# batd-htplus/intool-rag

Hardware: AMD Instinct MI355X
Metric: queries/sec, exact top-10 inner-product search, 1M x 1024-d fp32 index (higher is better)
Workload: dtype bf16 x bf16 -> f32 filter scan, f64 re-score of the f32 rows; 1 GPU; configs[1]: 1M x 1024-d synthetic unit vectors, brute-force inner-product top-10; rows=1000000, dim=1024, k=10, queries_per_pass=64, exchange=none, steps_in_flight=4, world=1, backend=none, allgather_payload_bytes_per_rank=0

## Files before the change

### intool-rag_amd/csrc/dense_plan.h

```cpp
#pragma once
#include <algorithm>
#include <cmath>
#include <cstddef>
#include <cstdint>

#include "../../include/hiprag.h"

namespace hiprag {

constexpr int kPassQ = 64;
constexpr int kMaxQ = 1024;
constexpr int kMaxKFast = 128;
constexpr int kClasses = 64;
constexpr int kNoFilterGroups = 1024;

constexpr int kStageHalf = 896;
constexpr int kThetaBack = 8;
constexpr int kCandBytes = 16;

constexpr int kWideBlocks = 8;
constexpr int kWideQTiles = 8;
constexpr int kWideKP = 4;
constexpr int kWideBufFrags = (kWideBlocks + kWideQTiles) * kWideKP * 64;
constexpr size_t kWideLds = (size_t)2 * kWideBufFrags * 16;
constexpr int kWideMinCus = 32;
constexpr int kWideMinQ = 256;

constexpr int kPipeSpareCus = 48;
constexpr int kPipeSpareCusWide = 32;

constexpr double kLaunchPasses = 4.0;
constexpr double kLaunchRefBytes = 4.096e9;
constexpr int kMinLaunchPasses = 4;

enum ScanMode : int {
    kScanQ64 = 2,
    kScanBf16 = 3,
};

using ScanShape = hipidx_scan_shape_t;

struct ScanPlan {
    bool run = false;
    bool wide = false;
    int waves = 8;
    int ring = 16;
    bool multi_pass = false;
    bool filter = false;
    int ncls = 1;
    size_t lds_bytes = 0;
    bool qtile_image = false;
};

inline int64_t ceil_div(int64_t a, int64_t b) { return (a + b - 1) / b; }

inline bool filter_on(const ScanShape& s) { return 2 * s.nblocks > kNoFilterGroups; }
inline bool uses_qtile_images(const ScanShape& s) { return s.mode == kScanBf16; }

inline int scan_waves(const ScanShape& s, int cus)
{
    return (s.mode == kScanBf16 && s.P % 32 == 0 && s.nblocks < (int64_t)cus * 8 * 9) ? 4 : 8;
}

inline bool wide_launch_on(const ScanShape& s, int nq, int cus)
{
    if (s.mode != kScanBf16 || s.wide_env == 0 || !filter_on(s) || cus < kWideMinCus) return false;
    if (s.wide_env == 1) return nq > kPassQ;
    return nq >= kWideMinQ && ceil_div(s.nblocks, kWideBlocks) >= cus;
}

inline int64_t stream_bytes_per_pass(const ScanShape& s) { return s.nblocks * s.P * (s.mode == kScanBf16 ? 512 : 1024); }
inline int64_t bytes_per_pass(const ScanShape& s, int metric, bool wide = false)
{
    return (stream_bytes_per_pass(s) + (metric == HIPRAG_METRIC_L2 ? s.nblocks * 32 * 4 : 0)) / (wide ? 4 : 1);
}

inline int launch_queries(const ScanShape& s)
{
    if (s.launch_env > 0) return std::max(kPassQ, std::min(kMaxQ, s.launch_env / kPassQ * kPassQ));
    ScanShape t = s;
    t.nblocks = std::max<int64_t>(s.nblocks, 1);
    const int np = (int)std::lround(kLaunchPasses * kLaunchRefBytes / (double)stream_bytes_per_pass(t));
    return std::max(kMinLaunchPasses, std::min(kMaxQ / kPassQ, np)) * kPassQ;
}

inline int pipe_spare_cus(const ScanShape& s, int launch_q)
{
    const int g48 = std::max(1, s.n_cu - kPipeSpareCus), g32 = std::max(1, s.n_cu - kPipeSpareCusWide);
    if (!wide_launch_on(s, launch_q, g48) || !wide_launch_on(s, launch_q, g32)) return kPipeSpareCus;
    const int64_t nrt = ceil_div(s.nblocks, kWideBlocks);
    return ceil_div(nrt, g32) < ceil_div(nrt, g48) ? kPipeSpareCusWide : kPipeSpareCus;
}

inline ScanPlan plan_scan(const ScanShape& s, int nq, int k, int cus)
{
    ScanPlan p;
    p.filter = filter_on(s);
    p.run = s.nblocks > 0 && k <= kMaxKFast;
    if (!p.run) return p;
    p.wide = wide_launch_on(s, nq, cus);
    p.waves = p.wide ? 8 : scan_waves(s, cus);
    p.multi_pass = nq > kPassQ;
    p.ring = p.wide ? 0 : (s.mode == kScanQ64 || (s.P / 2) % 16 == 0) ? 16 : 8;
    const int64_t bpw = ceil_div(s.nblocks, (int64_t)cus * p.waves);
    p.ncls = (int)std::max<int64_t>(1, std::min<int64_t>(kClasses, ceil_div(s.nblocks, bpw)));
    p.lds_bytes = p.wide ? kWideLds : (size_t)s.P * 1024 + (size_t)2 * kStageHalf * kCandBytes + 64 + (size_t)kThetaBack * 64 * 4;
    p.qtile_image = uses_qtile_images(s) && p.multi_pass;
    return p;
}

}
```

### intool-rag_amd/csrc/scan_wide.h

```cpp
#pragma once

constexpr int kWideQ = kWideQTiles * 32;
constexpr unsigned long long kWideWaitTicks = 20000ull;

constexpr int kWideBatch = 16;
constexpr int kWidePhaseT = kClasses / kWideBatch + 1;
constexpr int kWidePhaseA = kWidePhaseT + 1;

struct WidePend {
    float f[4][2], s[4][2];
    u32 mn;
    int64_t rt;
    int unit;
    int phase;
};
struct WideFlight {
    u32 ld[kWideBatch];
    u32 tc;
    u32 pos0, pos1;
};

__device__ __forceinline__ u32 wide_theta_fresh(const ScanArgs& a, int unit, int lane, bool live)
{
    u32 m = 0;
    if (live) {
        u32* s = a.slots + (size_t)unit * kClasses * 64 + lane;
        u32 mn = 0xFFFFFFFFu;
#pragma unroll 16
        for (int c = 0; c < kClasses; ++c) mn = min(mn, load_memside_u32(s + c * 64));
        if (mn != 0) atomicMax(a.thetac + unit * 64 + lane, mn);
        m = mn;
    }
    return m;
}

__device__ __forceinline__ void wide_test(const ScanArgs& a, const WidePend& P, int bh, int lane, u32 m, bool (&p0)[4], bool (&p1)[4])
{
    const int b = lane & 31;
    const u32 th0 = (u32)__shfl((int)m, b), th1 = (u32)__shfl((int)m, 32 + b);
    const int q0 = P.unit * 64 + b, q1 = q0 + 32;
    const int64_t blk0 = P.rt * kWideBlocks + 4 * bh;
#pragma unroll
    for (int i = 0; i < 4; ++i) {
        const bool there = blk0 + i < a.nblocks;
        p0[i] = there && q0 < a.nq && ord32(P.f[i][0]) >= th0;
        p1[i] = there && q1 < a.nq && ord32(P.f[i][1]) >= th1;
    }
}

__device__ __forceinline__ void wide_issue(const ScanArgs& a, const WidePend& P, WideFlight& X, int bh, int lane)
{
    const bool live = P.unit * 64 + lane < a.nq;
#pragma unroll
    for (int i = 0; i < kWideBatch; ++i) X.ld[i] = 0xFFFFFFFFu;
    X.tc = X.pos0 = X.pos1 = 0;
    if (P.phase < kWidePhaseT) {
        if (live) {
            const u32* sl = a.slots + ((size_t)P.unit * kClasses + (size_t)(P.phase - 1) * kWideBatch) * 64 + lane;
#pragma unroll
            for (int i = 0; i < kWideBatch; ++i) X.ld[i] = load_agent_u32(sl + i * 64);
        }
    }
    if (P.phase == kWidePhaseT) {
        if (live) X.tc = __hip_atomic_fetch_max(a.thetac + P.unit * 64 + lane, P.mn, __ATOMIC_RELAXED, __HIP_MEMORY_SCOPE_AGENT);
    }
    if (P.phase == kWidePhaseA) {
        bool p0[4], p1[4];
        wide_test(a, P, bh, lane, P.mn, p0, p1);
        const u32 n0 = (u32)p0[0] + (u32)p0[1] + (u32)p0[2] + (u32)p0[3], n1 = (u32)p1[0] + (u32)p1[1] + (u32)p1[2] + (u32)p1[3];
        const int q0 = P.unit * 64 + (lane & 31);
        if (n0) X.pos0 = atomicAdd(a.count + q0, n0);
        if (n1) X.pos1 = atomicAdd(a.count + q0 + 32, n1);
    }
}

__device__ __forceinline__ void wide_land(const ScanArgs& a, WidePend& P, const WideFlight& X, int bh, int lane)
{
#pragma unroll
    for (int i = 0; i < kWideBatch; ++i) P.mn = min(P.mn, X.ld[i]);
    if (P.phase == kWidePhaseT) {
        const bool live = P.unit * 64 + lane < a.nq;
        u32 m = live ? max(P.mn, X.tc) : 0u;
        if (__ballot(live && m == 0)) {
            const unsigned long long t0 = wall_clock64();
            for (int it = 0;; ++it) {
                if (live && m == 0) m = load_memside_u32(a.thetac + P.unit * 64 + lane);
                if (it && __ballot(live && m == 0)) m = max(m, wide_theta_fresh(a, P.unit, lane, live && m == 0));
                if (!__ballot(live && m == 0)) break;
                if (wall_clock64() - t0 > kWideWaitTicks) break;
                __builtin_amdgcn_s_sleep(127);
            }
        }
        P.mn = m;
    }
    if (P.phase == kWidePhaseA) {
        bool p0[4], p1[4];
        wide_test(a, P, bh, lane, P.mn, p0, p1);
        const int h = lane >> 5;
        const u32 q0 = (u32)(P.unit * 64 + (lane & 31)), q1 = q0 + 32;
        const int64_t blk0 = P.rt * kWideBlocks + 4 * bh;
        u32 pos0 = X.pos0, pos1 = X.pos1;
#pragma unroll
        for (int i = 0; i < 4; ++i) {
            const u32 gid = (u32)(2 * (blk0 + i) + h);
            if (p0[i]) {
                if (pos0 < (u32)kCandCap) a.list[(size_t)q0 * kCandCap + pos0] = Cand{pack_key(P.f[i][0], gid), P.s[i][0], q0};
                ++pos0;
            }
            if (p1[i]) {
                if (pos1 < (u32)kCandCap) a.list[(size_t)q1 * kCandCap + pos1] = Cand{pack_key(P.f[i][1], gid), P.s[i][1], q1};
                ++pos1;
            }
        }
    }
    P.phase = P.phase == kWidePhaseA ? 0 : P.phase + 1;
}

__device__ __forceinline__ void wide_drain(const ScanArgs& a, WidePend& P, int bh, int lane)
{
    while (P.phase) {
        WideFlight X;
        wide_issue(a, P, X, bh, lane);
        wide_land(a, P, X, bh, lane);
    }
}

template <int METRIC>
__device__ __forceinline__ void wide_park(const ScanArgs& a, const f32x16 (&acc)[4][2], WidePend& P, int64_t rt, int unit, int bh, int lane)
{
    const int h = lane >> 5;
    const int64_t blk0 = rt * kWideBlocks + 4 * bh;
    if (blk0 >= a.nblocks) return;
    float pm0 = -INFINITY, pm1 = -INFINITY;
#pragma unroll
    for (int i = 0; i < 4; ++i) {
        const int64_t blk = blk0 + i;
        P.f[i][0] = P.f[i][1] = P.s[i][0] = P.s[i][1] = -FLT_MAX;
        if (blk < a.nblocks) {
            f32x4 nrm[4];
            if (METRIC == HIPRAG_METRIC_L2) {
#pragma unroll
                for (int g = 0; g < 4; ++g) nrm[g] = *reinterpret_cast<const f32x4*>(a.norms + blk * kRowsPerBlock + 8 * g + 4 * h);
            }
            P.f[i][0] = block_lane_top2<METRIC>(acc[i][0], nrm, blk, h, a, P.s[i][0]);
            P.f[i][1] = block_lane_top2<METRIC>(acc[i][1], nrm, blk, h, a, P.s[i][1]);
            pm0 = fmaxf(pm0, P.f[i][0]);
            pm1 = fmaxf(pm1, P.f[i][1]);
        }
    }
    {
        const float x0 = fmaxf(pm0, __shfl_xor(pm0, 32)), x1 = fmaxf(pm1, __shfl_xor(pm1, 32));
        const float v = lane < 32 ? x0 : x1;
        const int cls = (int)((2 * rt + bh) & (kClasses - 1));
        if (unit * 64 + lane < a.nq) atomicMax(a.slots + ((size_t)unit * kClasses + cls) * 64 + lane, ord32(v));
    }
    P.mn = 0xFFFFFFFFu;
    P.rt = rt;
    P.unit = unit;
    P.phase = 1;
}

template <int METRIC>
__global__ __launch_bounds__(512) void scan_wide_kernel(ScanArgs a)
{
    extern __shared__ float4 qs[];
    const int tid = threadIdx.x, lane = tid & 63;
    const int wave = __builtin_amdgcn_readfirstlane(tid >> 6);
    __builtin_amdgcn_s_setprio(3);
    const int64_t gw = (int64_t)blockIdx.x * 8 + wave;
    if (a.stamps && lane == 0) a.stamps[2 * gw] = wall_clock64();
    if (a.gate && tid == 0) {
        const unsigned long long was = __hip_atomic_fetch_add(a.started, 1ull, __ATOMIC_RELAXED, __HIP_MEMORY_SCOPE_AGENT);
        if (was + 1 == a.target) __hip_atomic_fetch_max(a.gate, a.seq, __ATOMIC_RELAXED, __HIP_MEMORY_SCOPE_AGENT);
    }
    const int P2 = a.P / 2;
    const int KS = P2 / kWideKP;
    const int nunits = (a.nq + 63) / 64;
    const int ncol = (a.nq + kWideQ - 1) / kWideQ;
    const int64_t nrt = (a.nblocks + kWideBlocks - 1) / kWideBlocks;
    const int bh = wave & 1, qp = wave >> 1;
    const bf16x8* xh = reinterpret_cast<const bf16x8*>(a.xh);
    const bf16x8* qimg = reinterpret_cast<const bf16x8*>(a.qtile);
    bf16x8* lds = reinterpret_cast<bf16x8*>(qs);

    auto stage = [&](int64_t rt, int col, int ks, int buf) {
        bf16x8* dst = lds + buf * kWideBufFrags;
#pragma unroll
        for (int i = 0; i < 8; ++i) {
            const int c = wave + 8 * i;
            const int pc = ks * kWideKP + (c & 3);
            if (i < 4) {
                const int64_t blk = min(rt * kWideBlocks + (c >> 2), a.nblocks - 1);
                __builtin_amdgcn_global_load_lds((const void*)(xh + ((size_t)blk * P2 + pc) * 64 + lane), (scan_lds_ptr_t)(dst + c * 64), 16, 0, 0);
            } else {
                const int qt = col * kWideQTiles + ((c - 32) >> 2);
                if ((qt >> 1) < nunits)
                    __builtin_amdgcn_global_load_lds((const void*)(qimg + ((size_t)qt * P2 + pc) * 64 + lane), (scan_lds_ptr_t)(dst + c * 64), 16, 0, 0);
            }
        }
    };

    f32x16 acc[4][2];
    WidePend P;
    P.phase = 0;
    int64_t rt = blockIdx.x;
    int col = 0, ks = 0, buf = 0;
    bool have = rt < nrt;
    if (have) stage(rt, 0, 0, 0);
    while (have) {
        int64_t nr = rt;
        int nc = col, nk = ks + 1;
        if (nk == KS) {
            nk = 0;
            if (++nc == ncol) { nc = 0; nr += gridDim.x; }
        }
        const bool more = nr < nrt;
        asm volatile("s_waitcnt vmcnt(0)" ::: "memory");
        __syncthreads();
        int lane_e = lane;
        asm volatile("" : "+v"(lane_e));
        const bool pend = P.phase != 0;
        WideFlight X;
        if (pend) wide_issue(a, P, X, bh, lane_e);
        if (more) stage(nr, nc, nk, buf ^ 1);
        const int unit = col * (kWideQTiles / 2) + qp;
        if (unit < nunits) {
            if (ks == 0) {
#pragma unroll
                for (int i = 0; i < 4; ++i)
#pragma unroll
                    for (int e = 0; e < 16; ++e) { acc[i][0][e] = 0.f; acc[i][1][e] = 0.f; }
            }
            const bf16x8* A = lds + buf * kWideBufFrags + (4 * bh) * kWideKP * 64 + lane;
            const bf16x8* B = lds + buf * kWideBufFrags + (kWideBlocks + 2 * qp) * kWideKP * 64 + lane;
#pragma unroll
            for (int pc = 0; pc < kWideKP; ++pc) {
                bf16x8 av[4], bv[2];
#pragma unroll
                for (int i = 0; i < 4; ++i) av[i] = A[(i * kWideKP + pc) * 64];
#pragma unroll
                for (int j = 0; j < 2; ++j) bv[j] = B[(j * kWideKP + pc) * 64];
#pragma unroll
                for (int i = 0; i < 4; ++i) {
                    acc[i][0] = __builtin_amdgcn_mfma_f32_32x32x16_bf16(av[i], bv[0], acc[i][0], 0, 0, 0);
                    acc[i][1] = __builtin_amdgcn_mfma_f32_32x32x16_bf16(av[i], bv[1], acc[i][1], 0, 0, 0);
                }
            }
        }
        __builtin_amdgcn_sched_barrier(0);
        if (pend) wide_land(a, P, X, bh, lane_e);
        if (unit < nunits && ks == KS - 1) {
            wide_drain(a, P, bh, lane_e);
            wide_park<METRIC>(a, acc, P, rt, unit, bh, lane_e);
        }
        rt = nr; col = nc; ks = nk; have = more; buf ^= 1;
    }
    asm volatile("s_waitcnt vmcnt(0)" ::: "memory");
    wide_drain(a, P, bh, lane);
    if (a.stamps && lane == 0) a.stamps[2 * gw + 1] = wall_clock64();
}
```

Measured before the change: 391,900 queries/s.

## Replace wide-scan double buffer with deep separate row and query LDS rings

The wide scan kernel moves from a two-buffer LDS scheme with a full vmcnt(0) wait each step to separate multi-slot rings for index rows (5 slots) and query tiles (3 slots), with the k-piece per step halved. Loads are kept several steps ahead with partial vmcnt waits, LDS reads are hand-scheduled with inline ds_read and lgkmcnt waits interleaved with MFMAs, and the threshold and count atomics are issued as inline asm with counted waits, running only every other k-step. The goal is to hide global-memory latency and overlap the bookkeeping atomics with compute. In exchange the vmcnt accounting becomes fragile and depends on exact instruction counts, and theta refreshes arrive later, which can weaken filtering.

```diff
diff --git a/intool-rag_amd/csrc/dense_plan.h b/intool-rag_amd/csrc/dense_plan.h
--- a/intool-rag_amd/csrc/dense_plan.h
+++ b/intool-rag_amd/csrc/dense_plan.h
@@ -20,9 +20,13 @@
 
 constexpr int kWideBlocks = 8;
 constexpr int kWideQTiles = 8;
-constexpr int kWideKP = 4;
-constexpr int kWideBufFrags = (kWideBlocks + kWideQTiles) * kWideKP * 64;
-constexpr size_t kWideLds = (size_t)2 * kWideBufFrags * 16;
+constexpr int kWideKP = 2;
+constexpr int kWideBufFrags = kWideBlocks * kWideKP * 64;
+static_assert(kWideBlocks == kWideQTiles, "one slot size serves both rings");
+constexpr int kWideRowRing = 5;
+constexpr int kWideQRing = 3;
+constexpr size_t kWideLds = (size_t)(kWideRowRing + kWideQRing) * kWideBufFrags * 16;
+static_assert(kWideLds == 131072, "eight 16 KiB slots, one LDS object");
 constexpr int kWideMinCus = 32;
 constexpr int kWideMinQ = 256;
 
diff --git a/intool-rag_amd/csrc/scan_wide.h b/intool-rag_amd/csrc/scan_wide.h
--- a/intool-rag_amd/csrc/scan_wide.h
+++ b/intool-rag_amd/csrc/scan_wide.h
@@ -6,6 +6,18 @@
 constexpr int kWideBatch = 16;
 constexpr int kWidePhaseT = kClasses / kWideBatch + 1;
 constexpr int kWidePhaseA = kWidePhaseT + 1;
+constexpr int kWidePhaseEvery = 2;
+
+#define WIDE_DSR(dst, addr, off) asm volatile("ds_read_b128 %0, %1 offset:%2" : "=v"(dst) : "v"(addr), "n"(off) : "memory")
+#define WIDE_LGKM1(n, x) asm volatile("s_waitcnt lgkmcnt(%[c])" : "+v"(x) : [c] "n"(n) : "memory")
+#define WIDE_LGKM3(n, x, y, z) asm volatile("s_waitcnt lgkmcnt(%[c])" : "+v"(x), "+v"(y), "+v"(z) : [c] "n"(n) : "memory")
+
+#define WIDE_BAR()                                \
+    do {                                          \
+        __builtin_amdgcn_sched_barrier(0);        \
+        __builtin_amdgcn_s_barrier();             \
+        __builtin_amdgcn_sched_barrier(0);        \
+    } while (0)
 
 struct WidePend {
     float f[4][2], s[4][2];
@@ -20,6 +32,25 @@
     u32 pos0, pos1;
 };
 
+template <int I>
+__device__ __forceinline__ void wide_slot_loads(WideFlight& X, const u32* sl)
+{
+    asm volatile("global_load_dword %0, %1, off offset:%2 sc1" : "=v"(X.ld[I]) : "v"(sl), "n"(I * 256) : "memory");
+    if constexpr (I + 1 < kWideBatch) wide_slot_loads<I + 1>(X, sl);
+}
+__device__ __forceinline__ void wide_fetch_max(u32& out, u32* p, u32 v)
+{
+    asm volatile("global_atomic_umax %0, %1, %2, off sc0" : "=v"(out) : "v"(p), "v"(v) : "memory");
+}
+__device__ __forceinline__ void wide_fetch_add(u32& out, u32* p, u32 v)
+{
+    asm volatile("global_atomic_add %0, %1, %2, off sc0" : "=v"(out) : "v"(p), "v"(v) : "memory");
+}
+#define WIDE_WAIT1(younger, a) asm volatile("s_waitcnt vmcnt(%[n])" : "+v"(a) : [n] "n"(younger) : "memory")
+#define WIDE_WAIT2(younger, a, b) asm volatile("s_waitcnt vmcnt(%[n])" : "+v"(a), "+v"(b) : [n] "n"(younger) : "memory")
+#define WIDE_WAIT8(younger, r, o) \
+    asm volatile("s_waitcnt vmcnt(%[n])" : "+v"(r[o]), "+v"(r[o + 1]), "+v"(r[o + 2]), "+v"(r[o + 3]), "+v"(r[o + 4]), "+v"(r[o + 5]), "+v"(r[o + 6]), "+v"(r[o + 7]) : [n] "n"(younger) : "memory")
+
 __device__ __forceinline__ u32 wide_theta_fresh(const ScanArgs& a, int unit, int lane, bool live)
 {
     u32 m = 0;
@@ -51,35 +82,39 @@
 __device__ __forceinline__ void wide_issue(const ScanArgs& a, const WidePend& P, WideFlight& X, int bh, int lane)
 {
     const bool live = P.unit * 64 + lane < a.nq;
-#pragma unroll
-    for (int i = 0; i < kWideBatch; ++i) X.ld[i] = 0xFFFFFFFFu;
-    X.tc = X.pos0 = X.pos1 = 0;
+    const int ql = P.unit * 64 + (live ? lane : 0);
     if (P.phase < kWidePhaseT) {
-        if (live) {
-            const u32* sl = a.slots + ((size_t)P.unit * kClasses + (size_t)(P.phase - 1) * kWideBatch) * 64 + lane;
-#pragma unroll
-            for (int i = 0; i < kWideBatch; ++i) X.ld[i] = load_agent_u32(sl + i * 64);
-        }
+        wide_slot_loads<0>(X, a.slots + ((size_t)P.unit * kClasses + (size_t)(P.phase - 1) * kWideBatch) * 64 + (ql & 63));
     }
     if (P.phase == kWidePhaseT) {
-        if (live) X.tc = __hip_atomic_fetch_max(a.thetac + P.unit * 64 + lane, P.mn, __ATOMIC_RELAXED, __HIP_MEMORY_SCOPE_AGENT);
+        wide_fetch_max(X.tc, a.thetac + ql, live ? P.mn : 0u);
     }
     if (P.phase == kWidePhaseA) {
         bool p0[4], p1[4];
         wide_test(a, P, bh, lane, P.mn, p0, p1);
         const u32 n0 = (u32)p0[0] + (u32)p0[1] + (u32)p0[2] + (u32)p0[3], n1 = (u32)p1[0] + (u32)p1[1] + (u32)p1[2] + (u32)p1[3];
         const int q0 = P.unit * 64 + (lane & 31);
-        if (n0) X.pos0 = atomicAdd(a.count + q0, n0);
-        if (n1) X.pos1 = atomicAdd(a.count + q0 + 32, n1);
-    }
-}
-
-__device__ __forceinline__ void wide_land(const ScanArgs& a, WidePend& P, const WideFlight& X, int bh, int lane)
-{
-#pragma unroll
-    for (int i = 0; i < kWideBatch; ++i) P.mn = min(P.mn, X.ld[i]);
+        X.pos0 = X.pos1 = 0;
+        if (n0) wide_fetch_add(X.pos0, a.count + q0, n0);
+        if (n1) wide_fetch_add(X.pos1, a.count + q0 + 32, n1);
+    }
+}
+
+template <bool DRAIN>
+__device__ __forceinline__ void wide_land(const ScanArgs& a, WidePend& P, WideFlight& X, int bh, int lane)
+{
+    constexpr int YOUNGER = DRAIN ? 0 : 4;
+    const bool live = P.unit * 64 + lane < a.nq;
+    if (P.phase < kWidePhaseT) {
+        WIDE_WAIT8(YOUNGER, X.ld, 0);
+        WIDE_WAIT8(YOUNGER, X.ld, 8);
+        if (live) {
+#pragma unroll
+            for (int i = 0; i < kWideBatch; ++i) P.mn = min(P.mn, X.ld[i]);
+        }
+    }
     if (P.phase == kWidePhaseT) {
-        const bool live = P.unit * 64 + lane < a.nq;
+        WIDE_WAIT1(YOUNGER, X.tc);
         u32 m = live ? max(P.mn, X.tc) : 0u;
         if (__ballot(live && m == 0)) {
             const unsigned long long t0 = wall_clock64();
@@ -94,6 +129,7 @@
         P.mn = m;
     }
     if (P.phase == kWidePhaseA) {
+        WIDE_WAIT2(YOUNGER, X.pos0, X.pos1);
         bool p0[4], p1[4];
         wide_test(a, P, bh, lane, P.mn, p0, p1);
         const int h = lane >> 5;
@@ -121,7 +157,7 @@
     while (P.phase) {
         WideFlight X;
         wide_issue(a, P, X, bh, lane);
-        wide_land(a, P, X, bh, lane);
+        wide_land<true>(a, P, X, bh, lane);
     }
 }
 
@@ -183,77 +219,106 @@
     const bf16x8* qimg = reinterpret_cast<const bf16x8*>(a.qtile);
     bf16x8* lds = reinterpret_cast<bf16x8*>(qs);
 
-    auto stage = [&](int64_t rt, int col, int ks, int buf) {
-        bf16x8* dst = lds + buf * kWideBufFrags;
-#pragma unroll
-        for (int i = 0; i < 8; ++i) {
-            const int c = wave + 8 * i;
-            const int pc = ks * kWideKP + (c & 3);
-            if (i < 4) {
-                const int64_t blk = min(rt * kWideBlocks + (c >> 2), a.nblocks - 1);
-                __builtin_amdgcn_global_load_lds((const void*)(xh + ((size_t)blk * P2 + pc) * 64 + lane), (scan_lds_ptr_t)(dst + c * 64), 16, 0, 0);
-            } else {
-                const int qt = col * kWideQTiles + ((c - 32) >> 2);
-                if ((qt >> 1) < nunits)
-                    __builtin_amdgcn_global_load_lds((const void*)(qimg + ((size_t)qt * P2 + pc) * 64 + lane), (scan_lds_ptr_t)(dst + c * 64), 16, 0, 0);
-            }
-        }
+    auto advance = [&](int64_t& rt, int& col, int& ks) -> bool {
+        if (++ks < KS) return false;
+        ks = 0;
+        if (++col == ncol) { col = 0; rt += gridDim.x; }
+        return true;
+    };
+    struct Stream { const bf16x8* p; u32 d; };
+    auto row_stream = [&](int64_t rt) {
+        const int64_t b0 = min(rt * kWideBlocks + (wave >> 1), a.nblocks - 1);
+        const int64_t b1 = min(rt * kWideBlocks + (wave >> 1) + 4, a.nblocks - 1);
+        return Stream{xh + ((size_t)b0 * P2 + (wave & 1)) * 64, (u32)(b1 - b0) * (u32)P2 * 64u};
+    };
+    auto query_stream = [&](int col) {
+        const int t0 = min(col * kWideQTiles + (wave >> 1), 2 * nunits - 1);
+        const int t1 = min(col * kWideQTiles + (wave >> 1) + 4, 2 * nunits - 1);
+        return Stream{qimg + ((size_t)t0 * P2 + (wave & 1)) * 64, (u32)(t1 - t0) * (u32)P2 * 64u};
+    };
+    auto stage = [&](const Stream& S, int slot) {
+        bf16x8* dst = lds + slot * kWideBufFrags + wave * 64;
+        __builtin_amdgcn_global_load_lds((const void*)(S.p + lane), (scan_lds_ptr_t)dst, 16, 0, 0);
+        __builtin_amdgcn_global_load_lds((const void*)(S.p + S.d + lane), (scan_lds_ptr_t)(dst + 8 * 64), 16, 0, 0);
     };
 
     f32x16 acc[4][2];
     WidePend P;
     P.phase = 0;
     int64_t rt = blockIdx.x;
-    int col = 0, ks = 0, buf = 0;
-    bool have = rt < nrt;
-    if (have) stage(rt, 0, 0, 0);
-    while (have) {
-        int64_t nr = rt;
-        int nc = col, nk = ks + 1;
-        if (nk == KS) {
-            nk = 0;
-            if (++nc == ncol) { nc = 0; nr += gridDim.x; }
-        }
-        const bool more = nr < nrt;
-        asm volatile("s_waitcnt vmcnt(0)" ::: "memory");
-        __syncthreads();
-        int lane_e = lane;
-        asm volatile("" : "+v"(lane_e));
-        const bool pend = P.phase != 0;
-        WideFlight X;
-        if (pend) wide_issue(a, P, X, bh, lane_e);
-        if (more) stage(nr, nc, nk, buf ^ 1);
-        const int unit = col * (kWideQTiles / 2) + qp;
-        if (unit < nunits) {
-            if (ks == 0) {
-#pragma unroll
-                for (int i = 0; i < 4; ++i)
-#pragma unroll
-                    for (int e = 0; e < 16; ++e) { acc[i][0][e] = 0.f; acc[i][1][e] = 0.f; }
-            }
-            const bf16x8* A = lds + buf * kWideBufFrags + (4 * bh) * kWideKP * 64 + lane;
-            const bf16x8* B = lds + buf * kWideBufFrags + (kWideBlocks + 2 * qp) * kWideKP * 64 + lane;
-#pragma unroll
-            for (int pc = 0; pc < kWideKP; ++pc) {
-                bf16x8 av[4], bv[2];
-#pragma unroll
-                for (int i = 0; i < 4; ++i) av[i] = A[(i * kWideKP + pc) * 64];
-#pragma unroll
-                for (int j = 0; j < 2; ++j) bv[j] = B[(j * kWideKP + pc) * 64];
-#pragma unroll
-                for (int i = 0; i < 4; ++i) {
-                    acc[i][0] = __builtin_amdgcn_mfma_f32_32x32x16_bf16(av[i], bv[0], acc[i][0], 0, 0, 0);
-                    acc[i][1] = __builtin_amdgcn_mfma_f32_32x32x16_bf16(av[i], bv[1], acc[i][1], 0, 0, 0);
+    int col = 0, ks = 0;
+    if (rt < nrt) {
+        int64_t r_rt = rt, q_rt = rt;
+        int r_col = 0, r_ks = 0, q_col = 0, q_ks = 0;
+        Stream R = row_stream(r_rt), Q = query_stream(0);
+        auto next_rows = [&]() {
+            R.p += kWideKP * 64;
+            if (advance(r_rt, r_col, r_ks)) R = row_stream(r_rt);
+        };
+        auto next_queries = [&]() {
+            Q.p += kWideKP * 64;
+            if (advance(q_rt, q_col, q_ks)) Q = query_stream(q_col);
+        };
+        int rslot = 0, qslot = 0;
+        stage(R, 0); next_rows();
+        stage(R, 1); next_rows();
+        stage(Q, kWideRowRing + 0); next_queries();
+        stage(R, 2); next_rows();
+        stage(Q, kWideRowRing + 1); next_queries();
+        stage(R, 3); next_rows();
+        do {
+            asm volatile("s_waitcnt vmcnt(6)" ::: "memory");
+            WIDE_BAR();
+            int lane_e = lane;
+            asm volatile("" : "+v"(lane_e));
+            const bool pend = P.phase != 0 && (ks & (kWidePhaseEvery - 1)) == 0;
+            WideFlight X;
+            if (pend) wide_issue(a, P, X, bh, lane_e);
+            stage(Q, kWideRowRing + (qslot == 0 ? kWideQRing - 1 : qslot - 1));
+            stage(R, rslot == 0 ? kWideRowRing - 1 : rslot - 1);
+            next_queries();
+            next_rows();
+            const int unit = col * (kWideQTiles / 2) + qp;
+            if (unit < nunits) {
+                if (ks == 0) {
+#pragma unroll
+                    for (int i = 0; i < 4; ++i)
+#pragma unroll
+                        for (int e = 0; e < 16; ++e) { acc[i][0][e] = 0.f; acc[i][1][e] = 0.f; }
                 }
-            }
-        }
-        __builtin_amdgcn_sched_barrier(0);
-        if (pend) wide_land(a, P, X, bh, lane_e);
-        if (unit < nunits && ks == KS - 1) {
-            wide_drain(a, P, bh, lane_e);
-            wide_park<METRIC>(a, acc, P, rt, unit, bh, lane_e);
-        }
-        rt = nr; col = nc; ks = nk; have = more; buf ^= 1;
+                static_assert(kWideKP == 2, "the read order below is written out for two pieces per k-step");
+                const unsigned A = (unsigned)(uintptr_t)(scan_lds_ptr_t)(lds + rslot * kWideBufFrags + (4 * bh) * kWideKP * 64 + lane);
+                const unsigned B = (unsigned)(uintptr_t)(scan_lds_ptr_t)(lds + (kWideRowRing + qslot) * kWideBufFrags + (2 * qp) * kWideKP * 64 + lane);
+                bf16x8 a0, a1, a2, a3, b0, b1, c0, c1;
+#define WIDE_PAIR(i, av, q0, q1)                                                                 \
+                acc[i][0] = __builtin_amdgcn_mfma_f32_32x32x16_bf16(av, q0, acc[i][0], 0, 0, 0); \
+                acc[i][1] = __builtin_amdgcn_mfma_f32_32x32x16_bf16(av, q1, acc[i][1], 0, 0, 0)
+                WIDE_DSR(b0, B, 0); WIDE_DSR(b1, B, 2048);
+                WIDE_DSR(a0, A, 0); WIDE_DSR(a1, A, 2048); WIDE_DSR(a2, A, 4096); WIDE_DSR(a3, A, 6144);
+                WIDE_LGKM3(3, b0, b1, a0); WIDE_PAIR(0, a0, b0, b1);
+                WIDE_DSR(c0, B, 1024);
+                WIDE_LGKM1(3, a1); WIDE_PAIR(1, a1, b0, b1);
+                WIDE_DSR(c1, B, 3072);
+                WIDE_LGKM1(3, a2); WIDE_PAIR(2, a2, b0, b1);
+                WIDE_DSR(a0, A, 1024);
+                WIDE_LGKM1(3, a3); WIDE_PAIR(3, a3, b0, b1);
+                WIDE_DSR(a1, A, 3072); WIDE_DSR(a2, A, 5120); WIDE_DSR(a3, A, 7168);
+                WIDE_LGKM3(3, c0, c1, a0); WIDE_PAIR(0, a0, c0, c1); __builtin_amdgcn_sched_barrier(0);
+                WIDE_LGKM1(2, a1); WIDE_PAIR(1, a1, c0, c1); __builtin_amdgcn_sched_barrier(0);
+                WIDE_LGKM1(1, a2); WIDE_PAIR(2, a2, c0, c1); __builtin_amdgcn_sched_barrier(0);
+                WIDE_LGKM1(0, a3); WIDE_PAIR(3, a3, c0, c1);
+#undef WIDE_PAIR
+            }
+            __builtin_amdgcn_sched_barrier(0);
+            if (pend) wide_land<false>(a, P, X, bh, lane_e);
+            if (unit < nunits && ks == KS - 1) {
+                wide_drain(a, P, bh, lane_e);
+                wide_park<METRIC>(a, acc, P, rt, unit, bh, lane_e);
+            }
+            advance(rt, col, ks);
+            rslot = rslot == kWideRowRing - 1 ? 0 : rslot + 1;
+            qslot = qslot == kWideQRing - 1 ? 0 : qslot + 1;
+        } while (rt < nrt);
     }
     asm volatile("s_waitcnt vmcnt(0)" ::: "memory");
     wide_drain(a, P, bh, lane);
```

New measurement: 407,600 queries/s, median of 6. +4.0%, better.
